# ablab/spades

Hardware: NVIDIA H100
Metric: Mk-mers/s (extract+count+index) k=55, 150 bp reads (higher is better)
Workload: dtype u64

## Files before the change

spades_b200/csrc/count.cu:

```cuda
#include <algorithm>
#include <chrono>
#include <memory>

#include "pass_plan.h"
#include "sgpu_internal.h"

namespace sg {

__device__ __forceinline__ void prefetch_l2(const void *p) { asm volatile("prefetch.global.L2 [%0];" ::"l"(p)); }

struct ReadsSrc {
    const uint64_t *words;
    const uint64_t *offs;
    const uint32_t *lens;
    int64_t n;
    uint64_t nwords;
    int K;
    static constexpr int kIds = 24;
    static constexpr int kIdLines = 48;
    static constexpr bool kSubRanges = true;
    __device__ __forceinline__ uint64_t first_word(int64_t item) const { return offs[item]; }
    __device__ __forceinline__ uint32_t len(int64_t item) const { return lens[item]; }
    __device__ __forceinline__ void prefetch_items(int64_t item, int lane) const {
        if (lane == 0) prefetch_l2(lens + item);
// ... 213 lines not shown
        uint32_t unif = 0;
        bool staged = false;
        const bool has_next = t + kRollWarps < t1;
        const int64_t nx = (t + kRollWarps) * kRollTile;
        uint64_t next_w0 = 0;
        if (has_next) {
            next_w0 = src.first_word(nx);
            src.prefetch_items(nx, lane);
        }
        const uint32_t nunits = roll_warp_setup<BOTH>(src, item0, nitems, rw, &unif, &staged);
        uint64_t *row = ids ? reinterpret_cast<uint64_t *>(ids + tile_off[t]) : nullptr;
        for (uint32_t u = lane; u < nunits; u += 32) {
            const RollUnit q = roll_unit<BOTH>(rw, nitems, u, unif, K);
            const uint64_t *seq = staged ? static_cast<const uint64_t *>(rw.words + rw.off[q.it]) : src.words + src.first_word(item0 + q.it);
            RollState<NW> st;
            roll_init<NW>(st, seq, q.j0, K, q.cnt);
            const int nrec = BOTH ? 2 * q.cnt : q.cnt;
#pragma unroll 1
            for (int g = 0; g < Src::kIds / 4; ++g) {
                uint64_t acc = 0;
#pragma unroll
                for (int e = 0; e < 4; ++e) {
                    const int s = 4 * g + e;
                    uint32_t id = 0xffffu;
                    if (s < nrec) {
                        if (s > 0 && !(BOTH && (e & 1))) roll_next<NW>(st, K);
                        const Kmer<NW> k = BOTH ? ((e & 1) ? st.r : st.f) : kmer_is_minimal<NW>(st.f, st.r) ? st.f : st.r;
                        uint32_t part;
                        if (part_of<NW>(p, k, &part)) { atomicAdd(&hist[part], 1u); id = part; }
                    }
                    acc |= (uint64_t)id << (16 * e);
                }
                if (row) row[(size_t)u * (Src::kIds / 4) + g] = acc;
            }
        }
        if (has_next && lane < 10 && next_w0 + 16 * lane < src.nwords) prefetch_l2(src.words + next_w0 + 16 * lane);
        __syncwarp();
    }
    __syncthreads();
    uint32_t *out = blk_counts + (size_t)blockIdx.x * p.PA;
    for (uint32_t i = threadIdx.x; i < p.PA; i += blockDim.x) out[i] += hist[i];
}

static const uint32_t kABatchMin = 1024;
static_assert(kABatchMin / kRollWarps >= 32 * 2, "a warp's share of the smallest batch holds one window of a warp step");
__host__ __device__ __forceinline__ size_t abatch_offset(uint32_t PA) {
    return ((((size_t)2 * PA * 4 + 15) & ~(size_t)15) + (size_t)kRollWarps * sizeof(RollWarp) + 15) & ~(size_t)15;
}
template <int NW, bool PLANNED>
constexpr size_t abatch_rec_bytes() { return NW * sizeof(uint64_t) + (PLANNED ? sizeof(uint16_t) : sizeof(uint32_t) + sizeof(uint16_t)); }

static const uint32_t kABatchNoTag = 0xffffffffu;
static const int kABatchPartBits = 13;
template <int NW, class Src, bool BOTH>
__global__ void __launch_bounds__(kRollThreads, 2) levelA_scatter_roll_k(Src src, LevelA p, uint64_t *__restrict__ base, uint64_t *__restrict__ out,
                                                                        uint32_t row_stride, uint32_t cap) {
    extern __shared__ __align__(16) unsigned char sm_raw[];
    __shared__ uint32_t s_fill;
    __shared__ uint32_t warp_tot[kRollWarps];
    const uint32_t PA = p.PA;
    uint32_t *cur = reinterpret_cast<uint32_t *>(sm_raw);
    uint32_t *cnt = cur + PA;
    RollWarp &rw = *roll_warp_slice(sm_raw, 2 * PA);
    uint64_t *stage = reinterpret_cast<uint64_t *>(sm_raw + abatch_offset(PA));
    uint32_t *tags = reinterpret_cast<uint32_t *>(stage + (size_t)cap * NW);
    uint16_t *idx = reinterpret_cast<uint16_t *>(tags + cap);
    uint64_t *mybase = base + (size_t)blockIdx.x * row_stride;
    const uint64_t region0 = mybase[0];
    for (uint32_t i = threadIdx.x; i < PA; i += blockDim.x) { cur[i] = (uint32_t)(mybase[i] - region0); cnt[i] = 0; }
    if (threadIdx.x == 0) s_fill = 0;
    __syncthreads();
    uint64_t *const out0 = out + region0 * NW;
    const int K = p.K;
    const int lane = threadIdx.x & 31, warp = threadIdx.x >> 5;
    const uint32_t lt_mask = (1u << lane) - 1u;
    const int64_t ntiles = (src.n + kRollTile - 1) / kRollTile;
    const int64_t per = (ntiles + gridDim.x - 1) / gridDim.x;
    const int64_t t0 = (int64_t)blockIdx.x * per, t1 = min(ntiles, t0 + per);

    int64_t t = t0 + warp;
    bool need_setup = true;
    int nitems = 0;
    uint32_t nunits = 0, unif = 0;
    bool staged = false;
    uint64_t next_w0 = 0;
    int u = 0, s = 0, cnt_w = 0;
    RollState<NW> st;
    for (;;) {
        while (t < t1) {
            if (need_setup) {
                const int64_t item0 = t * kRollTile;
                nitems = (int)min((int64_t)kRollTile, src.n - item0);
                const int64_t nx = (t + kRollWarps) * kRollTile;
                if (t + kRollWarps < t1) {
                    next_w0 = src.first_word(nx);
                    src.prefetch_items(nx, lane);
                }
                nunits = roll_warp_setup<BOTH>(src, item0, nitems, rw, &unif, &staged);
                u = lane - 32; s = cnt_w = 0;
                need_setup = false;
            }
            if (s >= cnt_w && u < (int)nunits) {
                u += 32;
                if (u < (int)nunits) {
                    const RollUnit q = roll_unit<BOTH>(rw, nitems, (uint32_t)u, unif, K);
                    const uint64_t *seq = staged ? static_cast<const uint64_t *>(rw.words + rw.off[q.it]) : src.words + src.first_word(t * kRollTile + q.it);
                    roll_init<NW>(st, seq, q.j0, K, q.cnt);
                    s = 0; cnt_w = BOTH ? 2 * q.cnt : q.cnt;
                }
// ... 18 lines not shown
            const uint32_t bal = __ballot_sync(0xffffffffu, mine);
            if (bal) {
                const uint32_t n = __popc(bal);
                uint32_t b0 = 0;
                if (lane == 0) b0 = atomicAdd(&s_fill, n);
                b0 = __shfl_sync(0xffffffffu, b0, 0);
                if (b0 + n > cap) {
                    if (b0 < cap && (uint32_t)lane < cap - b0) tags[b0 + lane] = kABatchNoTag;
                    break;
                }
                if (mine) {
                    const uint32_t i = b0 + __popc(bal & lt_mask);
                    const uint32_t rank = atomicAdd(&cnt[part], 1u) & 0xffffu;
                    store_rec<NW>(stage + (size_t)i * NW, k);
                    tags[i] = (rank << kABatchPartBits) | part;
                }
            }
            if (act && ++s < cnt_w && (!BOTH || !(s & 1))) roll_next<NW>(st, K);
        }
        const bool more = __syncthreads_or(t < t1);
        const uint32_t nslots = min(s_fill, cap);
        const uint32_t own = (PA + kRollThreads - 1) / kRollThreads;
        const uint32_t j0 = min(PA, threadIdx.x * own), j1 = min(PA, j0 + own);
        uint32_t sum = 0;
        for (uint32_t j = j0; j < j1; ++j) sum += cnt[j] & 0xffffu;
        uint32_t inc = sum;
#pragma unroll
        for (int o = 1; o < 32; o <<= 1) {
            const uint32_t v = __shfl_up_sync(0xffffffffu, inc, o);
            if (lane >= o) inc += v;
        }
        if (lane == 31) warp_tot[warp] = inc;
        __syncthreads();
        uint32_t wb = 0, total = 0;
#pragma unroll
        for (int w = 0; w < kRollWarps; ++w) { const uint32_t v = warp_tot[w]; if (w < warp) wb += v; total += v; }
        uint32_t o = wb + inc - sum;
        for (uint32_t j = j0; j < j1; ++j) {
            const uint32_t c = cnt[j] & 0xffffu;
            o += c;
            cnt[j] = o << 16;
            cur[j] += c;
        }
        if (threadIdx.x == 0) s_fill = 0;
        __syncthreads();
        for (uint32_t i = threadIdx.x; i < nslots; i += kRollThreads) {
            const uint32_t tg = tags[i];
            if (tg == kABatchNoTag) continue;
            idx[(cnt[tg & ((1u << kABatchPartBits) - 1)] >> 16) - 1 - (tg >> kABatchPartBits)] = (uint16_t)i;
        }
        __syncthreads();
        for (uint32_t q = threadIdx.x; q < total; q += kRollThreads) {
            const uint32_t i = idx[q], tg = tags[i];
            const uint32_t slot = cur[tg & ((1u << kABatchPartBits) - 1)] - 1 - (tg >> kABatchPartBits);
            store_rec_stream<NW>(out0 + (size_t)slot * NW, load_rec<NW>(stage + (size_t)i * NW));
        }
        __syncthreads();
        if (!more) break;
    }
    for (uint32_t i = threadIdx.x; i < PA; i += blockDim.x) mybase[i] = region0 + cur[i];
}

template <int NW, class Src, bool BOTH>
__global__ void __launch_bounds__(kRollThreads, 2) levelA_scatter_plan_k(Src src, LevelA p, uint64_t *__restrict__ base, uint64_t *__restrict__ out,
                                                                        const uint64_t *__restrict__ tile_off, const uint16_t *__restrict__ ids,
                                                                        uint32_t id_lo, uint32_t row_stride, uint32_t q_lo, uint64_t ids_len, uint32_t cap) {
    extern __shared__ __align__(16) unsigned char sm_raw[];
    __shared__ uint32_t warp_tot[kRollWarps];
    constexpr int kR = BOTH ? 2 : 1;
    constexpr int kRowV = Src::kIds / 8;
    const uint32_t PA = p.PA;
    uint32_t *cur = reinterpret_cast<uint32_t *>(sm_raw);
    uint32_t *run = cur + PA;
    RollWarp &rw = *roll_warp_slice(sm_raw, 2 * PA);
    uint64_t *stage = reinterpret_cast<uint64_t *>(sm_raw + abatch_offset(PA));
    uint16_t *ptag = reinterpret_cast<uint16_t *>(stage + (size_t)cap * NW);
    uint64_t *mybase = base + (size_t)blockIdx.x * row_stride + q_lo;
    const uint64_t region0 = mybase[0];
    for (uint32_t i = threadIdx.x; i < PA; i += blockDim.x) { cur[i] = (uint32_t)(mybase[i] - region0); run[i] = 0; }
    __syncthreads();
    uint64_t *const out0 = out + region0 * NW;
    const int K = p.K;
    const int lane = threadIdx.x & 31, warp = threadIdx.x >> 5;
    const int64_t ntiles = (src.n + kRollTile - 1) / kRollTile;
    const int64_t per = (ntiles + gridDim.x - 1) / gridDim.x;
    const int64_t t0 = (int64_t)blockIdx.x * per, t1 = min(ntiles, t0 + per);
    const uint32_t share = cap / kRollWarps;

    int64_t pt = t0 + warp;
    int pj = 0, ps = 0;
    uint32_t pn = 0;
    bool p_enter = true;
    const ulonglong2 *prow = nullptr;
    int64_t rt = pt;
    int rj = 0, rs = 0;
    bool need_setup = true;
    int nitems = 0;
    uint32_t nunits = 0, unif = 0;
    bool staged = false;
    uint64_t next_w0 = 0;
    const ulonglong2 *row = nullptr;
    for (;;) {
        uint32_t room = share;
        while (pt < t1) {
            if (p_enter) {
                const uint64_t a = tile_off[pt], b = tile_off[pt + 1];
                if (pt + kRollWarps < t1) {
                    const uint64_t nr = tile_off[pt + kRollWarps];
                    if ((Src::kIdLines >= 32 || lane < Src::kIdLines) && nr + 64 * lane < ids_len) prefetch_l2(ids + nr + 64 * lane);
                    if (lane < Src::kIdLines - 32 && nr + 64 * (32 + lane) < ids_len) prefetch_l2(ids + nr + 64 * (32 + lane));
                }
                pn = (uint32_t)((b - a) / Src::kIds);
                prow = reinterpret_cast<const ulonglong2 *>(ids + a);
                p_enter = false;
            }
            if ((uint32_t)pj * 32 >= pn) {
                pt += kRollWarps; pj = 0; ps = 0; p_enter = true;
                continue;
            }
// ... 68 lines not shown
                __syncwarp();
                rt += kRollWarps; rj = 0; rs = 0;
                need_setup = true;
                continue;
            }
            const int end = (rt == pt && rj == pj) ? ps : Src::kIds;
            const int u = rj * 32 + lane;
            if (u < (int)nunits) {
                const RollUnit q = roll_unit<BOTH>(rw, nitems, (uint32_t)u, unif, K);
                const int s_end = min(end, BOTH ? 2 * q.cnt : q.cnt);
                if (rs < s_end) {
                    uint64_t idq[Src::kIds / 4];
#pragma unroll
                    for (int v = 0; v < kRowV; ++v) {
                        const ulonglong2 x = __ldg(row + (size_t)u * kRowV + v);
                        idq[2 * v] = x.x; idq[2 * v + 1] = x.y;
                    }
                    for (int w = 0; w < rs / 4; ++w) {
#pragma unroll
                        for (int v = 0; v + 1 < Src::kIds / 4; ++v) idq[v] = idq[v + 1];
                    }
                    idq[0] >>= 16 * (rs & 3);
                    const uint64_t *seq = staged ? static_cast<const uint64_t *>(rw.words + rw.off[q.it]) : src.words + src.first_word(rt * kRollTile + q.it);
                    RollState<NW> st;
                    roll_init<NW>(st, seq, q.j0 + rs / kR, K, q.cnt - rs / kR);
                    for (int s = rs;;) {
                        const uint32_t part = (uint32_t)(idq[0] & 0xffffu) - id_lo;
                        if (part < PA) {
                            const bool fwd = BOTH ? !(s & 1) : kmer_is_minimal<NW>(st.f, st.r);
                            Kmer<NW> k;
#pragma unroll
                            for (int j = 0; j < NW; ++j) k.w[j] = fwd ? st.f.w[j] : st.r.w[j];
                            const uint32_t pos = atomicAdd(&run[part], 1u << 16) >> 16;
                            store_rec<NW>(stage + (size_t)pos * NW, k);
                            ptag[pos] = (uint16_t)part;
                        }
                        if (++s >= s_end) break;
                        if (!BOTH || !(s & 1)) roll_next<NW>(st, K);
                        if ((s & 3) == 0) {
#pragma unroll
                            for (int v = 0; v + 1 < Src::kIds / 4; ++v) idq[v] = idq[v + 1];
                        } else {
                            idq[0] >>= 16;
                        }
                    }
                }
            }
            if (end == Src::kIds) { ++rj; rs = 0; } else rs = end;
        }
        __syncthreads();
        for (uint32_t q = threadIdx.x; q < total; q += kRollThreads) {
            const uint32_t part = ptag[q];
            const uint32_t slot = cur[part] - (run[part] >> 16) + q;
            store_rec_stream<NW>(out0 + (size_t)slot * NW, load_rec<NW>(stage + (size_t)q * NW));
        }
        if (!more) break;
    }
    for (uint32_t i = threadIdx.x; i < PA; i += blockDim.x) mybase[i] = region0 + cur[i];
}

struct Seg {
    uint64_t start;
    uint64_t len;
    uint32_t bits;
    uint32_t bb;
};

__global__ void seg_init_k(const uint64_t *__restrict__ part_start, const uint64_t *__restrict__ part_total, uint32_t PA, int rA,
                           uint32_t b_lo, Seg *__restrict__ segs) {
    uint32_t part = blockIdx.x * blockDim.x + threadIdx.x;
    if (part >= PA) return;
    Seg s;
    s.start = part_start[part]; s.len = part_total[part]; s.bits = (uint32_t)rA; s.bb = ((b_lo + (part >> rA)) << 1) | 0u;
    segs[part] = s;
}

struct Pieces {
    const uint64_t *pbase;
    const uint32_t *cnt;
    uint32_t cnt_stride, PA;
    int G;
};
static const int kMaxPieces = 1024;

__global__ void stage_rows_k(const uint32_t *__restrict__ cnt, uint32_t cnt_stride, uint32_t PA, uint64_t *__restrict__ rel, uint64_t *__restrict__ row_total) {
    __shared__ uint64_t wsum[8];
    __shared__ uint64_t carry_s;
    const uint32_t *row = cnt + (size_t)blockIdx.x * cnt_stride;
    uint64_t *out = rel + (size_t)blockIdx.x * PA;
    const int lane = threadIdx.x & 31, warp = threadIdx.x >> 5;
    if (threadIdx.x == 0) carry_s = 0;
    __syncthreads();
    for (uint32_t b = 0; b < PA; b += blockDim.x) {
        const uint32_t i = b + threadIdx.x;
        const uint64_t v = i < PA ? row[i] : 0;
        uint64_t inc = v;
#pragma unroll
        for (int o = 1; o < 32; o <<= 1) {
            uint64_t t = __shfl_up_sync(0xffffffffu, inc, o);
            if (lane >= o) inc += t;
        }
        if (lane == 31) wsum[warp] = inc;
        __syncthreads();
        uint64_t wb = 0, all = 0;
        for (int w = 0; w < 8; ++w) { if (w < warp) wb += wsum[w]; all += wsum[w]; }
        const uint64_t carry = carry_s;
        if (i < PA) out[i] = carry + wb + inc - v;
        __syncthreads();
        if (threadIdx.x == 0) carry_s = carry + all;
        __syncthreads();
    }
    if (threadIdx.x == 0) row_total[blockIdx.x] = carry_s;
}
__global__ void stage_add_k(uint64_t *__restrict__ rel, const uint64_t *__restrict__ row_start, uint32_t PA, int G) {
    const uint64_t i = (uint64_t)blockIdx.x * blockDim.x + threadIdx.x;
    if (i >= (uint64_t)G * PA) return;
    rel[i] += row_start[i / PA];
}

struct RefinePlan { uint32_t cap, target, rmax; int total_bits; };
__device__ __forceinline__ int plan_r(const RefinePlan &rp, uint64_t len, uint32_t bits) {
    if (len <= rp.cap) return 0;
    int rem = rp.total_bits - (int)bits;
    if (rem <= 0) return 0;
    uint64_t want = (len + rp.target - 1) / rp.target;
    int r = 1;
    while (r < (int)rp.rmax && (1ull << r) < want) ++r;
    return r < rem ? r : rem;
}
__global__ void refine_plan_k(const Seg *__restrict__ segs, uint64_t n, RefinePlan rp, uint32_t *__restrict__ nchild, uint32_t *__restrict__ isw, int force_all) {
    uint64_t i = (uint64_t)blockIdx.x * blockDim.x + threadIdx.x;
    if (i >= n) return;
    int r = plan_r(rp, segs[i].len, segs[i].bits);
    nchild[i] = r ? (1u << r) : 1u;
    isw[i] = (r || force_all) ? 1u : 0u;
}
__global__ void refine_copy_k(const Seg *__restrict__ segs, uint64_t n, const uint32_t *__restrict__ isw, const uint64_t *__restrict__ child_base,
                              const uint64_t *__restrict__ work_pos, Seg *__restrict__ nsegs, uint64_t *__restrict__ worklist) {
    uint64_t i = (uint64_t)blockIdx.x * blockDim.x + threadIdx.x;
    if (i >= n) return;
    if (isw[i]) worklist[work_pos[i]] = i;
    else nsegs[child_base[i]] = segs[i];
}

static const int kRThreads = 1024;
static const int kRWarps = kRThreads / 32;
static const int kRMaxBins = 2048;
template <int NW> struct RBatch {
    static const int RPT = NW == 1 ? 12 : NW == 2 ? 8 : NW == 3 ? 4 : 3;
    static const int N = RPT * kRThreads;
    static constexpr size_t smem() { return (size_t)N * (NW * sizeof(uint64_t) + sizeof(uint32_t)); }
};

template <int NW, bool PIECED>
__global__ void __launch_bounds__(kRThreads) refine_k(const Seg *__restrict__ segs, const uint64_t *__restrict__ worklist, uint64_t nwork,
                                                     const uint64_t *__restrict__ child_base, RefinePlan rp, int K,
                                                     uint64_t *__restrict__ buf0, uint64_t *__restrict__ buf1, Seg *__restrict__ nsegs,
                                                     unsigned long long *__restrict__ work_counter, Pieces pc) {
    constexpr int RPT = RBatch<NW>::RPT, N = RBatch<NW>::N;
    __shared__ uint32_t hist[kRMaxBins];
    __shared__ uint32_t run_off[kRMaxBins];
    __shared__ uint32_t run_slot[kRMaxBins];
    __shared__ uint32_t warp_tot[kRWarps];
    __shared__ unsigned long long s_w;
    __shared__ uint64_t pc_start[PIECED ? kMaxPieces : 1];
    __shared__ uint32_t pc_len[PIECED ? kMaxPieces : 1];
    extern __shared__ uint64_t sm_refine_dyn[];
    uint64_t *stage = sm_refine_dyn;
    uint32_t *stage_slot = reinterpret_cast<uint32_t *>(stage + (size_t)N * NW);
    const int lane = threadIdx.x & 31, warp = threadIdx.x >> 5;
    for (;;) {
        if (threadIdx.x == 0) s_w = atomicAdd(work_counter, 1ull);
        __syncthreads();
        const uint64_t wi = s_w;
        __syncthreads();
        if (wi >= nwork) return;
        const uint64_t si = worklist[wi];
        const Seg s = segs[si];
        const int r = plan_r(rp, s.len, s.bits);
        const uint32_t nb = 1u << r;
        const uint64_t *src = ((s.bb & 1) ? buf1 : buf0) + s.start * NW;
        uint64_t *dst = ((s.bb & 1) ? buf0 : buf1) + s.start * NW;
        if (PIECED) {
            for (int g = threadIdx.x; g < pc.G; g += blockDim.x) {
                pc_start[g] = pc.pbase[(size_t)g * pc.PA + si];
                pc_len[g] = pc.cnt[(size_t)g * pc.cnt_stride + si];
            }
        }
        for (uint32_t i = threadIdx.x; i < nb; i += blockDim.x) hist[i] = 0;
        __syncthreads();
        if (PIECED) {
            for (int g = warp; g < pc.G; g += kRWarps) {
                const uint64_t *ps = buf0 + pc_start[g] * NW;
                const uint32_t n = pc_len[g];
                uint32_t i = lane;
                for (; i + 96 < n; i += 128) {
                    const Kmer<NW> k0 = load_rec<NW>(ps + (uint64_t)i * NW), k1 = load_rec<NW>(ps + (uint64_t)(i + 32) * NW);
                    const Kmer<NW> k2 = load_rec<NW>(ps + (uint64_t)(i + 64) * NW), k3 = load_rec<NW>(ps + (uint64_t)(i + 96) * NW);
                    atomicAdd(&hist[key_bits<NW>(k0, K, (int)s.bits, r)], 1u);
                    atomicAdd(&hist[key_bits<NW>(k1, K, (int)s.bits, r)], 1u);
                    atomicAdd(&hist[key_bits<NW>(k2, K, (int)s.bits, r)], 1u);
                    atomicAdd(&hist[key_bits<NW>(k3, K, (int)s.bits, r)], 1u);
                }
                for (; i < n; i += 32) {
                    const Kmer<NW> k = load_rec<NW>(ps + (uint64_t)i * NW);
                    atomicAdd(&hist[key_bits<NW>(k, K, (int)s.bits, r)], 1u);
                }
            }
        } else {
            for (uint64_t i = threadIdx.x; i < s.len; i += blockDim.x) {
                Kmer<NW> k = load_rec<NW>(src + i * NW);
                atomicAdd(&hist[key_bits<NW>(k, K, (int)s.bits, r)], 1u);
            }
        }
        __syncthreads();
        uint32_t a = 0, b = 0;
        const uint32_t i0 = 2 * threadIdx.x;
        if (i0 < nb) { a = hist[i0]; hist[i0] = 0; }
        if (i0 + 1 < nb) { b = hist[i0 + 1]; hist[i0 + 1] = 0; }
        uint32_t v = a + b, inc = v;
#pragma unroll
        for (int o = 1; o < 32; o <<= 1) {
            uint32_t t = __shfl_up_sync(0xffffffffu, inc, o);
            if (lane >= o) inc += t;
        }
        if (lane == 31) warp_tot[warp] = inc;
        __syncthreads();
        if (warp == 0) {
            uint32_t w = warp_tot[lane], winc = w;
#pragma unroll
            for (int o = 1; o < 32; o <<= 1) {
                uint32_t t = __shfl_up_sync(0xffffffffu, winc, o);
                if (lane >= o) winc += t;
            }
            warp_tot[lane] = winc - w;
        }
        __syncthreads();
        const uint32_t ex = warp_tot[warp] + inc - v;
        const uint64_t cb = child_base[si];
        if (i0 < nb) {
            Seg c; c.start = s.start + ex; c.len = a; c.bits = s.bits + (uint32_t)r; c.bb = s.bb ^ 1u;
            nsegs[cb + i0] = c;
        }
        if (i0 + 1 < nb) {
// ... 26 lines not shown
                for (int j = 0; j < RPT; ++j) {
                    const uint64_t i = cpos + threadIdx.x + (uint64_t)kRThreads * j;
                    if (i < s.len) { rec[j] = load_rec<NW>(src + i * NW); have |= 1u << j; }
                }
                cpos += N;
            }
        };
        load_batch();
        for (;;) {
            uint32_t tag[RPT];
#pragma unroll
            for (int j = 0; j < RPT; ++j) {
                if (have >> j & 1u) {
                    const uint32_t bin = key_bits<NW>(rec[j], K, (int)s.bits, r);
                    tag[j] = (atomicAdd(&hist[bin], 1u) << 11) | bin;
                }
            }
            if (!__syncthreads_or(have)) break;
            const uint32_t c0 = i0 < nb ? hist[i0] : 0u, c1 = i0 + 1 < nb ? hist[i0 + 1] : 0u;
            const uint32_t bv = c0 + c1;
            uint32_t binc = bv;
#pragma unroll
            for (int o = 1; o < 32; o <<= 1) {
                uint32_t t = __shfl_up_sync(0xffffffffu, binc, o);
                if (lane >= o) binc += t;
            }
            if (lane == 31) warp_tot[warp] = binc;
            __syncthreads();
            uint32_t w = warp_tot[lane], winc = w;
#pragma unroll
            for (int o = 1; o < 32; o <<= 1) {
                uint32_t t = __shfl_up_sync(0xffffffffu, winc, o);
                if (lane >= o) winc += t;
            }
            const uint32_t total = __shfl_sync(0xffffffffu, winc, 31);
            const uint32_t off = __shfl_sync(0xffffffffu, winc - w, warp) + binc - bv;
            if (i0 < nb) { run_off[i0] = off; run_slot[i0] = cur0; hist[i0] = 0; cur0 += c0; }
            if (i0 + 1 < nb) { run_off[i0 + 1] = off + c0; run_slot[i0 + 1] = cur1; hist[i0 + 1] = 0; cur1 += c1; }
            __syncthreads();
#pragma unroll
            for (int j = 0; j < RPT; ++j) {
                if (have >> j & 1u) {
                    const uint32_t bin = tag[j] & (kRMaxBins - 1), rank = tag[j] >> 11;
                    const uint32_t p = run_off[bin] + rank;
                    store_rec<NW>(stage + (size_t)p * NW, rec[j]);
                    stage_slot[p] = run_slot[bin] + rank;
                }
            }
            load_batch();
            __syncthreads();
            for (uint32_t p = threadIdx.x; p < total; p += kRThreads)
                store_rec_stream<NW>(dst + (uint64_t)stage_slot[p] * NW, load_rec<NW>(stage + (size_t)p * NW));
        }
    }
}

template <int NW> struct SortCfg { static const int CAP = NW <= 2 ? 2048 : 1024; };
static const int kSThreads = 512;
static const int kSWarps = kSThreads / 32;

template <int NW>
__device__ __forceinline__ void lsd_pass(const uint64_t *A, uint64_t *Bf, uint32_t n, int K, int pos, int width, uint32_t *cnt ,
                                         uint32_t *tot ) {
    static_assert(kSThreads >= 256, "one thread per digit");
    const int lane = threadIdx.x & 31, warp = threadIdx.x >> 5;
    const uint32_t chunk = ((n + kSWarps * 32 - 1) / (kSWarps * 32)) * 32;
    const uint32_t w0 = warp * chunk;
    for (int i = threadIdx.x; i < kSWarps * 256; i += kSThreads) cnt[i] = 0;
    __syncthreads();
    for (uint32_t r = 0; r < chunk; r += 32) {
        const uint32_t i = w0 + r + lane;
        uint32_t d = 256;
        if (i < n) d = key_bits<NW>(load_rec<NW>(A + (size_t)i * NW), K, pos, width);
        const uint32_t m = __match_any_sync(0xffffffffu, d);
        if (d < 256 && (int)(__ffs(m) - 1) == lane) cnt[warp * 256 + d] += __popc(m);
        __syncwarp();
    }
    __syncthreads();
    {
        const uint32_t d = threadIdx.x;
        uint32_t run = 0, inc = 0;
        if (d < 256) {
#pragma unroll
            for (int w = 0; w < kSWarps; ++w) { uint32_t t = cnt[w * 256 + d]; cnt[w * 256 + d] = run; run += t; }
            inc = run;
#pragma unroll
            for (int o = 1; o < 32; o <<= 1) {
                uint32_t t = __shfl_up_sync(0xffffffffu, inc, o);
                if (lane >= o) inc += t;
            }
            if (lane == 31) tot[warp] = inc;
        }
        __syncthreads();
        if (d < 256) {
            uint32_t wb = 0;
            for (int w = 0; w < warp; ++w) wb += tot[w];
            const uint32_t ex = wb + inc - run;
#pragma unroll
            for (int w = 0; w < kSWarps; ++w) cnt[w * 256 + d] += ex;
        }
    }
    __syncthreads();
    for (uint32_t r = 0; r < chunk; r += 32) {
        const uint32_t i = w0 + r + lane;
        uint32_t d = 256;
        Kmer<NW> k;
// ... 393 lines not shown
struct KSetBuilder {
    Ctx *ctx;
    std::unique_ptr<KSet> ks;
    DArr<unsigned long long> d_bsz;
    int64_t first = 0;
    bool double_selfrc;
    std::unique_ptr<ResultSink> sink;
    KSetBuilder(Ctx *c, int K, int nw, int B, bool counts, bool double_selfrc_, bool on_host) : ctx(c), ks(new KSet()), double_selfrc(double_selfrc_) {
        ks->ctx = c; ks->K = K; ks->nw = nw; ks->B = B; ks->has_counts = counts; ks->on_host = on_host;
        if (on_host) sink.reset(new ResultSink(c, ks.get()));
        d_bsz.alloc(c, (size_t)B);
        SG_CUDA(cudaMemsetAsync(d_bsz.p, 0, (size_t)B * 8, c->stream));
    }
    Chunk &open(int b_lo, int b_hi, uint64_t n) {
        if (sink) sink->drain();
        ks->chunks.emplace_back();
        Chunk &ch = ks->chunks.back();
        ch.n = (int64_t)n; ch.b_lo = b_lo; ch.b_hi = b_hi; ch.first = first;
        ch.keys.alloc(ctx, (size_t)n * ks->nw + 2, true);
        if (ks->has_counts) ch.counts.alloc(ctx, (size_t)n + 1, true);
        return ch;
    }
    void close() {
        first += ks->chunks.back().n;
        if (sink) sink->push();
    }
    KSet *finish() {
        if (sink) { sink->drain(); sink.reset(); }
        const int B = ks->B;
        std::vector<unsigned long long> hb(B);
        SG_CUDA(cudaMemcpyAsync(hb.data(), d_bsz.p, (size_t)B * 8, cudaMemcpyDeviceToHost, ctx->stream));
        SG_CUDA(cudaStreamSynchronize(ctx->stream));
        ks->bsz.assign(B, 0); ks->bstart.assign(B + 1, 0);
        for (int b = 0; b < B; ++b) { ks->bsz[b] = (int64_t)hb[b]; ks->bstart[b + 1] = ks->bstart[b] + ks->bsz[b]; }
        ks->n = first;
        SG_CHECK(ks->bstart[B] == ks->n, 6, "internal: bucket sizes do not add up");
        return ks.release();
    }
};

template <int NW>
static void sort_pass(Ctx *ctx, int K, DArr<uint64_t> &X, DArr<uint64_t> &Y, const uint64_t *part_start_p, const uint64_t *part_total_p, uint32_t PA,
                      int rA_, uint32_t b_lo, int b_hi, KSetBuilder &set, Timer &tm, Trace &tr, const Pieces *pieces = nullptr) {
    constexpr int CAP = SortCfg<NW>::CAP;
    const int total_bits = 2 * K;
    cudaStream_t st = ctx->stream;
    uint64_t nsegs = PA;
    DArr<Seg> segs(ctx, nsegs);
    seg_init_k<<<div_up(PA, 256), 256, 0, st>>>(part_start_p, part_total_p, PA, rA_, b_lo, segs.p);
    ctx->launches++;
    RefinePlan rp; rp.cap = CAP; rp.target = sort_target<NW>(); rp.total_bits = total_bits;
    rp.rmax = tuning().rmax;
    DArr<unsigned long long> wcounter(ctx, 4);
    tm.start();
    uint64_t rounds = 0;
    for (int round = 0; round < 300; ++round) {
        DArr<uint32_t> nchild(ctx, nsegs + 1), isw(ctx, nsegs + 1);
        DArr<uint64_t> cbase(ctx, nsegs + 1), wpos(ctx, nsegs + 1);
        SG_CUDA(cudaMemsetAsync(nchild.p + nsegs, 0, 4, st));
        SG_CUDA(cudaMemsetAsync(isw.p + nsegs, 0, 4, st));
        const bool pieced = pieces && round == 0;
        refine_plan_k<<<div_up(nsegs, 256), 256, 0, st>>>(segs.p, nsegs, rp, nchild.p, isw.p, pieced ? 1 : 0);
        ctx->launches++;
        exclusive_scan_u32_to_u64(ctx, nchild.p, cbase.p, nsegs + 1);
        exclusive_scan_u32_to_u64(ctx, isw.p, wpos.p, nsegs + 1);
        uint64_t tot[2];
        SG_CUDA(cudaMemcpyAsync(&tot[0], cbase.p + nsegs, 8, cudaMemcpyDeviceToHost, st));
        SG_CUDA(cudaMemcpyAsync(&tot[1], wpos.p + nsegs, 8, cudaMemcpyDeviceToHost, st));
        SG_CUDA(cudaStreamSynchronize(st));
        if (tot[1] == 0) break;
        DArr<Seg> nsegs_arr(ctx, tot[0]);
        DArr<uint64_t> worklist(ctx, tot[1]);
        refine_copy_k<<<div_up(nsegs, 256), 256, 0, st>>>(segs.p, nsegs, isw.p, cbase.p, wpos.p, nsegs_arr.p, worklist.p);
        ctx->launches++;
        SG_CUDA(cudaMemsetAsync(wcounter.p, 0, 8, st));
        const int grid = (int)std::min<uint64_t>(tot[1], (uint64_t)ctx->num_sms);
        const size_t sm = RBatch<NW>::smem();
        if (pieced) {
            SG_CUDA(cudaFuncSetAttribute(refine_k<NW, true>, cudaFuncAttributeMaxDynamicSharedMemorySize, (int)sm));
            refine_k<NW, true><<<grid, kRThreads, sm, st>>>(segs.p, worklist.p, tot[1], cbase.p, rp, K, X.p, Y.p, nsegs_arr.p, wcounter.p, *pieces);
        } else {
            SG_CUDA(cudaFuncSetAttribute(refine_k<NW, false>, cudaFuncAttributeMaxDynamicSharedMemorySize, (int)sm));
            refine_k<NW, false><<<grid, kRThreads, sm, st>>>(segs.p, worklist.p, tot[1], cbase.p, rp, K, X.p, Y.p, nsegs_arr.p, wcounter.p, Pieces());
        }
        ctx->launches++;
        SG_CUDA(cudaGetLastError());
        tr.mark("refine round");
        (round == 0 ? ctx->times.refine_splits_round0 : ctx->times.refine_splits_later) += tot[0] - nsegs;
        ++rounds;
        segs = std::move(nsegs_arr);
        nsegs = tot[0];
    }
    ctx->times.refine_rounds_max = std::max(ctx->times.refine_rounds_max, rounds);
    ctx->times.refine += tm.stop();
    DArr<uint32_t> ndist(ctx, nsegs + 1);
    DArr<unsigned long long> stats(ctx, 4);
    SG_CUDA(cudaMemsetAsync(ndist.p, 0, ndist.bytes(), st));
    SG_CUDA(cudaMemsetAsync(stats.p, 0, 32, st));
    SG_CUDA(cudaMemsetAsync(wcounter.p, 0, 8, st));
    tm.start();
    {
        auto launch = [&](auto kernel, size_t smem) {
            SG_CUDA(cudaFuncSetAttribute(kernel, cudaFuncAttributeMaxDynamicSharedMemorySize, (int)smem));
            int occ = 1;
            SG_CUDA(cudaOccupancyMaxActiveBlocksPerMultiprocessor(&occ, kernel, kSThreads, smem));
            if (occ < 1) occ = 1;
            int grid = (int)std::min<uint64_t>(nsegs, (uint64_t)ctx->num_sms * occ);
            if (grid < 1) grid = 1;
            kernel<<<grid, kSThreads, smem, st>>>(segs.p, nsegs, K, X.p, Y.p, ndist.p, wcounter.p, stats.p);
        };
        launch(local_sort3_k<NW, kSortBinBits, CAP>, SortSmem<NW, kSortBinBits, CAP>::bytes);
        ctx->launches++;
        SG_CUDA(cudaGetLastError());
    }
    DArr<uint64_t> dbase(ctx, nsegs + 1);
    exclusive_scan_u32_to_u64(ctx, ndist.p, dbase.p, nsegs + 1);
    uint64_t D = 0;
    unsigned long long h_stats[4];
    SG_CUDA(cudaMemcpyAsync(&D, dbase.p + nsegs, 8, cudaMemcpyDeviceToHost, st));
    SG_CUDA(cudaMemcpyAsync(h_stats, stats.p, 32, cudaMemcpyDeviceToHost, st));
    SG_CUDA(cudaStreamSynchronize(st));
    ctx->times.local_sort += tm.stop();
    tr.mark("local sort");
    SG_CHECK(h_stats[0] == 0, 6, "internal: oversize segment with unfixed key bits reached the local sort");
    ctx->times.sort_lsd_fallbacks += h_stats[1];
    ctx->times.sort_oversize_equal += h_stats[2];
    Chunk &ch = set.open((int)b_lo, b_hi, D);
    tm.start();
    if (nsegs) {
        compact_k<NW><<<div_up((int64_t)nsegs * 32, 256), 256, 0, st>>>(segs.p, nsegs, ndist.p, dbase.p, X.p, Y.p, K, set.ks->has_counts ? 1 : 0,
                                                                     set.double_selfrc ? 1 : 0, ch.keys.p, ch.counts.p, set.d_bsz.p);
        ctx->launches++;
        SG_CUDA(cudaGetLastError());
    }
    ctx->times.compact += tm.stop();
    tr.mark("compact");
    set.close();
}

template <int NW, class Src, bool BOTH>
struct LevelAJob {
    Ctx *ctx = nullptr;
    std::vector<Src> srcs;
    int K = 0, B = 0, rA = 0, G = 0;
    int s_lo = 0, s_hi = 0;
    uint32_t PA_all = 0;
    bool use_ids = false;
// ... 55 lines not shown
static void levelA_count(LevelAJob<NW, Src, BOTH> &job, Timer &tm, Trace &tr) {
    Ctx *ctx = job.ctx;
    cudaStream_t st = ctx->stream;
    const uint32_t PA_all = job.PA_all;
    const int G = job.G;
    SG_CHECK(PA_all >= 1 && PA_all <= (uint32_t)kLevelAMaxParts, 6, "internal: level-A partition table too large");
    LevelA pa_all;
    pa_all.K = job.K; pa_all.B = (uint32_t)job.B; pa_all.b_lo = (uint32_t)job.s_lo; pa_all.b_hi = (uint32_t)job.s_hi; pa_all.rA = job.rA; pa_all.PA = PA_all;
    job.blk_counts.alloc(ctx, (size_t)G * PA_all);
    job.part_total_all.alloc(ctx, (size_t)PA_all + 1);
    job.h_part.assign(PA_all, 0);
    SG_CUDA(cudaMemsetAsync(job.blk_counts.p, 0, job.blk_counts.bytes(), st));
    job.tile_off.clear(); job.ids.clear();
    job.tile_off.resize(job.srcs.size()); job.ids.resize(job.srcs.size());
    const double free0 = (double)ctx->free_bytes();
    std::vector<uint64_t> nslots(job.srcs.size(), 0);
    uint64_t all_slots = 0;
    for (size_t si = 0; si < job.srcs.size(); ++si) {
        const Src &src = job.srcs[si];
        if (src.n == 0) continue;
        const int64_t ntiles = (src.n + kRollTile - 1) / kRollTile;
        DArr<uint32_t> ttot(ctx, (size_t)ntiles + 1);
        job.tile_off[si].alloc(ctx, (size_t)ntiles + 1);
        SG_CUDA(cudaMemsetAsync(ttot.p + ntiles, 0, 4, st));
        roll_tile_ids_k<BOTH><<<div_up(ntiles, 8), 256, 0, st>>>(src, ntiles, ttot.p);
        ctx->launches++;
        exclusive_scan_u32_to_u64(ctx, ttot.p, job.tile_off[si].p, (size_t)ntiles + 1);
        SG_CUDA(cudaMemcpyAsync(&nslots[si], job.tile_off[si].p + ntiles, 8, cudaMemcpyDeviceToHost, st));
        SG_CUDA(cudaStreamSynchronize(st));
        all_slots += nslots[si];
    }
    job.use_ids = PA_all < 0xffffu && (double)all_slots * 2.0 < free0 * 0.20;
    for (size_t si = 0; si < job.srcs.size(); ++si) {
        if (!job.use_ids) job.tile_off[si] = DArr<uint64_t>();
        else if (job.srcs[si].n) job.ids[si].alloc(ctx, (size_t)nslots[si] + 8);
    }
    tm.start();
    SG_CUDA(cudaFuncSetAttribute(levelA_count_roll_k<NW, Src, BOTH>, cudaFuncAttributeMaxDynamicSharedMemorySize, (int)roll_smem_bytes(PA_all)));
    job.for_each_src([&](size_t si, const Src &src) {
        levelA_count_roll_k<NW, Src, BOTH><<<G, kRollThreads, roll_smem_bytes(PA_all), st>>>(src, pa_all, job.blk_counts.p, job.tile_off[si].p, job.ids[si].p);
        ctx->launches++;
    });
    SG_CUDA(cudaGetLastError());
    levelA_totals_k<<<div_up(PA_all, 256), 256, 0, st>>>(job.blk_counts.p, PA_all, G, job.part_total_all.p);
    ctx->launches++;
    SG_CUDA(cudaMemcpyAsync(job.h_part.data(), job.part_total_all.p, (size_t)PA_all * 8, cudaMemcpyDeviceToHost, st));
    SG_CUDA(cudaStreamSynchronize(st));
    ctx->times.extract_count += tm.stop();
    tr.mark("A1 count+totals");
}

template <int NW, class Src, bool BOTH>
static void levelA_scatter(LevelAJob<NW, Src, BOTH> &job, int b_lo, int b_hi, uint64_t I_pass, uint64_t total_records, uint64_t *X, uint64_t *pbase_buf,
                           Pieces &pcs, Timer &tm, Trace &tr) {
    Ctx *ctx = job.ctx;
    cudaStream_t st = ctx->stream;
    const int G = job.G;
    const uint32_t PA_all = job.PA_all;
    const uint32_t p_lo = (uint32_t)(b_lo - job.s_lo) << job.rA;
    LevelA pa;
    pa.K = job.K; pa.B = (uint32_t)job.B; pa.b_lo = (uint32_t)b_lo; pa.b_hi = (uint32_t)b_hi; pa.rA = job.rA; pa.PA = (uint32_t)(b_hi - b_lo) << job.rA;
    const uint32_t PA = pa.PA;
    SG_CHECK(PA >= 1 && PA <= (uint32_t)kLevelAMaxParts && G <= kMaxPieces, 6, "internal: level-A pass geometry");
    DArr<uint64_t> base(ctx, (size_t)G * PA);
    {
        DArr<uint64_t> row_total(ctx, (size_t)G + 1), row_start(ctx, (size_t)G + 1);
        SG_CUDA(cudaMemsetAsync(row_total.p + G, 0, 8, st));
        stage_rows_k<<<G, 256, 0, st>>>(job.blk_counts.p + p_lo, PA_all, PA, base.p, row_total.p);
        exclusive_scan_u64(ctx, row_total.p, row_start.p, (size_t)G + 1);
        stage_add_k<<<div_up((int64_t)G * PA, 256), 256, 0, st>>>(base.p, row_start.p, PA, G);
        ctx->launches += 2;
        SG_CUDA(cudaMemcpyAsync(pbase_buf, base.p, (size_t)G * PA * 8, cudaMemcpyDeviceToDevice, st));
    }
    pcs.pbase = pbase_buf; pcs.cnt = job.blk_counts.p + p_lo; pcs.cnt_stride = PA_all; pcs.PA = PA; pcs.G = G;
    tm.start();
    int nsub_auto = (int)(4.0 * (double)I_pass / (double)std::max<uint64_t>(1, total_records) + 0.5);
    nsub_auto = std::min(4, std::max(1, nsub_auto));
    uint32_t nsub = job.use_ids && !BOTH && Src::kSubRanges ? (uint32_t)(tuning().a_sub ? tuning().a_sub : nsub_auto) : 1u;
    if (nsub > PA) nsub = PA;
    for (uint32_t sb = 0; sb < nsub; ++sb) {
        const uint32_t q_lo = (uint32_t)((uint64_t)PA * sb / nsub), q_hi = (uint32_t)((uint64_t)PA * (sb + 1) / nsub);
        if (q_hi == q_lo) continue;
        LevelA pa_sub = pa;
        pa_sub.PA = q_hi - q_lo;
        uint32_t cap = 0;
        const size_t smem = job.use_ids ? levelA_batch_smem<NW, true>(pa_sub.PA, &cap) : levelA_batch_smem<NW, false>(pa_sub.PA, &cap);
        if (job.use_ids) SG_CUDA(cudaFuncSetAttribute(levelA_scatter_plan_k<NW, Src, BOTH>, cudaFuncAttributeMaxDynamicSharedMemorySize, (int)smem));
        else SG_CUDA(cudaFuncSetAttribute(levelA_scatter_roll_k<NW, Src, BOTH>, cudaFuncAttributeMaxDynamicSharedMemorySize, (int)smem));
        job.for_each_src([&](size_t si, const Src &src) {
            if (job.use_ids)
                levelA_scatter_plan_k<NW, Src, BOTH><<<G, kRollThreads, smem, st>>>(src, pa_sub, base.p, X, job.tile_off[si].p, job.ids[si].p, p_lo + q_lo, PA, q_lo, (uint64_t)job.ids[si].n, cap);
            else
                levelA_scatter_roll_k<NW, Src, BOTH><<<G, kRollThreads, smem, st>>>(src, pa, base.p, X, PA, cap);
            ctx->launches++; ctx->times.level_a_scatters++;
        });
    }
    SG_CUDA(cudaGetLastError());
    ctx->times.extract_scatter += tm.stop();
    tr.mark("A2 scatter");
}

static double pass_bytes_needed(uint64_t recs, size_t W) { return (double)recs * W * 2.0 + (double)recs * (W + 4) * 0.6 + (64 << 20); }

template <int NW, bool BOTH, class Src>
static void run_count(Ctx *ctx, const std::vector<Src> &srcs, int K, uint64_t est_records, KSetBuilder &set, ChunkStager *stage = nullptr) {
    const int total_bits = 2 * K, B = set.ks->B;
    const size_t W = 8 * NW;
    cudaStream_t st = ctx->stream;
    Timer tm(st);
    Trace tr("sgpu count", st);

    const int rA = levelA_key_bits(est_records, B, total_bits, sort_target<NW>(), tuning().pa_max);
    ctx->times.level_a_key_bits = (uint64_t)rA;
    const int SR = std::max(1, kLevelAMaxParts >> rA);
    const int n_ranges = (B + SR - 1) / SR;
    for (int s_lo = 0; s_lo < B; s_lo += SR) {
        const int share = (kMaxChunks - (int)set.ks->chunks.size()) / (n_ranges - s_lo / SR);
        LevelAJob<NW, Src, BOTH> job;
        job.ctx = ctx; job.srcs = srcs; job.K = K; job.B = B; job.rA = rA; job.G = ctx->num_sms * levelA_ctas_per_sm(); job.stage = stage;
        job.s_lo = s_lo; job.s_hi = std::min(B, s_lo + SR);
        job.PA_all = (uint32_t)(job.s_hi - job.s_lo) << rA;
        levelA_count(job, tm, tr);
        std::vector<uint64_t> before(job.s_hi - job.s_lo + 1, 0);
        for (int b = job.s_lo; b < job.s_hi; ++b) before[b - job.s_lo + 1] = before[b - job.s_lo] + job.bucket_records(b);
        PassPlan plan(job.s_lo, job.s_hi, share, std::move(before));
        const uint64_t total_records = plan.records(job.s_lo, job.s_hi);
        auto need = [&](int a, int b) { return pass_bytes_needed(plan.records(a, b), W); };
        plan.aim((double)ctx->budget_left(), set.sink != nullptr, need, [&](int a, int b) { return (double)plan.records(a, b) * (W + 4) * 0.5; });
        while (!plan.done()) {
            const int b_lo = plan.bounds.back(), b_hi = plan.next((double)ctx->budget_left(), need);
            const uint64_t I = plan.records(b_lo, b_hi);
            const uint32_t p_lo = (uint32_t)(b_lo - job.s_lo) << rA;
            const uint32_t PA = (uint32_t)(b_hi - b_lo) << rA;
            DArr<uint64_t> part_total(ctx, PA + 1), part_start(ctx, PA + 1);
            SG_CUDA(cudaMemcpyAsync(part_total.p, job.part_total_all.p + p_lo, (size_t)PA * 8, cudaMemcpyDeviceToDevice, st));
            SG_CUDA(cudaMemsetAsync(part_total.p + PA, 0, 8, st));
            exclusive_scan_u64(ctx, part_total.p, part_start.p, PA + 1);
            ctx->times.passes++;
            ctx->times.instances += I;
            DArr<uint64_t> X(ctx, (size_t)I * NW + 2), Y(ctx, (size_t)I * NW + 2);
            DArr<uint64_t> pbase(ctx, (size_t)job.G * PA);
            Pieces pcs;
            levelA_scatter(job, b_lo, b_hi, I, total_records, X.p, pbase.p, pcs, tm, tr);
            sort_pass<NW>(ctx, K, X, Y, part_start.p, part_total.p, PA, rA, (uint32_t)b_lo, b_hi, set, tm, tr, &pcs);
        }
    }
}

__global__ void count_windows_k(const uint32_t *__restrict__ lens, int64_t n, int K, unsigned long long *__restrict__ out) {
    unsigned long long s = 0;
    for (int64_t i = (int64_t)blockIdx.x * blockDim.x + threadIdx.x; i < n; i += (int64_t)gridDim.x * blockDim.x) {
        int L = (int)lens[i];
        if (L >= K) s += (unsigned long long)(L - K + 1);
    }
    for (int o = 16; o; o >>= 1) s += __shfl_down_sync(0xffffffffu, s, o);
    if ((threadIdx.x & 31) == 0 && s) atomicAdd(out, s);
}

static uint64_t count_windows(Ctx *ctx, int K) {
    DArr<unsigned long long> d_w(ctx, 1);
    SG_CUDA(cudaMemsetAsync(d_w.p, 0, 8, ctx->stream));
    if (ctx->n_reads) {
        count_windows_k<<<ctx->num_sms * 4, 256, 0, ctx->stream>>>(ctx->d_lens, ctx->n_reads, K, d_w.p);
        ctx->launches++;
    }
    unsigned long long wn = 0;
    SG_CUDA(cudaMemcpyAsync(&wn, d_w.p, 8, cudaMemcpyDeviceToHost, ctx->stream));
    SG_CUDA(cudaStreamSynchronize(ctx->stream));
    return (uint64_t)wn;
}

static ReadsSrc reads_source(Ctx *ctx, int K) {
    ReadsSrc src;
    src.words = ctx->d_words; src.offs = ctx->d_offs; src.lens = ctx->d_lens; src.n = ctx->n_reads; src.nwords = ctx->n_words; src.K = K;
    return src;
}

template <int NW>
static KSet *count_reads_nw(Ctx *ctx, int K, int B, int mode, bool on_host) {
    ensure_reads_on_device(ctx);
    const uint64_t wn = count_windows(ctx, K);
    std::vector<ReadsSrc> srcs{reads_source(ctx, K)};
    const bool canonical = mode == kCanonical;
    KSetBuilder set(ctx, K, NW, B, canonical, canonical && K % 2 == 0, on_host);
    if (canonical) run_count<NW, false>(ctx, srcs, K, wn, set);
    else run_count<NW, true>(ctx, srcs, K, wn * 2, set);
    return set.finish();
}

KSet *count_from_reads(Ctx *ctx, int K, int B, int mode, bool result_on_host) {
    SG_CHECK(K >= 1 && K <= 128, 2, "K must be in [1,128]");
    SG_CHECK(B >= 1 && B <= (1 << 20), 2, "num_buckets must be in [1, 2^20]");
    ctx->times = PhaseTimes();
    switch (nwords_of(K)) {
        case 1: return count_reads_nw<1>(ctx, K, B, mode, result_on_host);
        case 2: return count_reads_nw<2>(ctx, K, B, mode, result_on_host);
// ... 484 lines not shown
```

Measured before the change: 8709.

## Build next-digit histograms during level-A scatter to skip refine's piece histogram pass

The level-A scatter kernels now atomically count, per partition, the next dw key bits of each record into a global digits table. The first refinement round then builds its bin histogram from this table instead of re-reading every scattered record piece. This is meant to remove a full read pass over the pass buffer at the cost of global atomics during scatter and an extra PA<<dw table. It also adds a device-side consistency flag with a host sync and a partition-size check.

```diff
diff --git a/spades_b200/csrc/count.cu b/spades_b200/csrc/count.cu
--- a/spades_b200/csrc/count.cu
+++ b/spades_b200/csrc/count.cu
@@ -289,9 +289,13 @@
 
 static const uint32_t kABatchNoTag = 0xffffffffu;
 static const int kABatchPartBits = 13;
+template <int NW>
+__device__ __forceinline__ uint32_t next_digit(const Kmer<NW> &k, int K, int rA, int w) {
+    return w ? (uint32_t)(k.w[0] >> ((NW == 1 ? 2 * K : 64) - rA - w)) & ((1u << w) - 1u) : 0u;
+}
 template <int NW, class Src, bool BOTH>
 __global__ void __launch_bounds__(kRollThreads, 2) levelA_scatter_roll_k(Src src, LevelA p, uint64_t *__restrict__ base, uint64_t *__restrict__ out,
-                                                                        uint32_t row_stride, uint32_t cap) {
+                                                                        uint32_t row_stride, uint32_t cap, uint32_t *__restrict__ digits, int dw) {
     extern __shared__ __align__(16) unsigned char sm_raw[];
     __shared__ uint32_t s_fill;
     __shared__ uint32_t warp_tot[kRollWarps];
@@ -416,8 +420,11 @@
         __syncthreads();
         for (uint32_t q = threadIdx.x; q < total; q += kRollThreads) {
             const uint32_t i = idx[q], tg = tags[i];
-            const uint32_t slot = cur[tg & ((1u << kABatchPartBits) - 1)] - 1 - (tg >> kABatchPartBits);
-            store_rec_stream<NW>(out0 + (size_t)slot * NW, load_rec<NW>(stage + (size_t)i * NW));
+            const uint32_t part = tg & ((1u << kABatchPartBits) - 1);
+            const uint32_t slot = cur[part] - 1 - (tg >> kABatchPartBits);
+            const Kmer<NW> k = load_rec<NW>(stage + (size_t)i * NW);
+            store_rec_stream<NW>(out0 + (size_t)slot * NW, k);
+            if (digits) atomicAdd(&digits[((size_t)part << dw) | next_digit<NW>(k, K, p.rA, dw)], 1u);
         }
         __syncthreads();
         if (!more) break;
@@ -428,7 +435,8 @@
 template <int NW, class Src, bool BOTH>
 __global__ void __launch_bounds__(kRollThreads, 2) levelA_scatter_plan_k(Src src, LevelA p, uint64_t *__restrict__ base, uint64_t *__restrict__ out,
                                                                         const uint64_t *__restrict__ tile_off, const uint16_t *__restrict__ ids,
-                                                                        uint32_t id_lo, uint32_t row_stride, uint32_t q_lo, uint64_t ids_len, uint32_t cap) {
+                                                                        uint32_t id_lo, uint32_t row_stride, uint32_t q_lo, uint64_t ids_len, uint32_t cap,
+                                                                        uint32_t *__restrict__ digits, int dw) {
     extern __shared__ __align__(16) unsigned char sm_raw[];
     __shared__ uint32_t warp_tot[kRollWarps];
     constexpr int kR = BOTH ? 2 : 1;
@@ -603,7 +611,9 @@
         for (uint32_t q = threadIdx.x; q < total; q += kRollThreads) {
             const uint32_t part = ptag[q];
             const uint32_t slot = cur[part] - (run[part] >> 16) + q;
-            store_rec_stream<NW>(out0 + (size_t)slot * NW, load_rec<NW>(stage + (size_t)q * NW));
+            const Kmer<NW> k = load_rec<NW>(stage + (size_t)q * NW);
+            store_rec_stream<NW>(out0 + (size_t)slot * NW, k);
+            if (digits) atomicAdd(&digits[((size_t)(q_lo + part) << dw) | next_digit<NW>(k, K, p.rA, dw)], 1u);
         }
         if (!more) break;
     }
@@ -629,8 +639,9 @@
 struct Pieces {
     const uint64_t *pbase;
     const uint32_t *cnt;
+    const uint32_t *digits;
     uint32_t cnt_stride, PA;
-    int G;
+    int G, dw;
 };
 static const int kMaxPieces = 1024;
 
@@ -707,7 +718,7 @@
 __global__ void __launch_bounds__(kRThreads) refine_k(const Seg *__restrict__ segs, const uint64_t *__restrict__ worklist, uint64_t nwork,
                                                      const uint64_t *__restrict__ child_base, RefinePlan rp, int K,
                                                      uint64_t *__restrict__ buf0, uint64_t *__restrict__ buf1, Seg *__restrict__ nsegs,
-                                                     unsigned long long *__restrict__ work_counter, Pieces pc) {
+                                                     unsigned long long *__restrict__ work_counter, Pieces pc, uint32_t *__restrict__ bad) {
     constexpr int RPT = RBatch<NW>::RPT, N = RBatch<NW>::N;
     __shared__ uint32_t hist[kRMaxBins];
     __shared__ uint32_t run_off[kRMaxBins];
@@ -740,7 +751,13 @@
         }
         for (uint32_t i = threadIdx.x; i < nb; i += blockDim.x) hist[i] = 0;
         __syncthreads();
-        if (PIECED) {
+        if (PIECED && pc.digits) {
+            const uint32_t *dg = pc.digits + (si << pc.dw);
+            for (uint32_t e = threadIdx.x; e < (1u << pc.dw); e += blockDim.x) {
+                const uint32_t v = dg[e];
+                if (v) atomicAdd(&hist[e >> (pc.dw - r)], v);
+            }
+        } else if (PIECED) {
             for (int g = warp; g < pc.G; g += kRWarps) {
                 const uint64_t *ps = buf0 + pc_start[g] * NW;
                 const uint32_t n = pc_len[g];
@@ -873,6 +890,7 @@
             for (uint32_t p = threadIdx.x; p < total; p += kRThreads)
                 store_rec_stream<NW>(dst + (uint64_t)stage_slot[p] * NW, load_rec<NW>(stage + (size_t)p * NW));
         }
+        if ((i0 < nb && cur0 != ex + a) || (i0 + 1 < nb && cur1 != ex + a + b)) *bad = 1u;
     }
 }
 
@@ -1372,6 +1390,8 @@
     RefinePlan rp; rp.cap = CAP; rp.target = sort_target<NW>(); rp.total_bits = total_bits;
     rp.rmax = tuning().rmax;
     DArr<unsigned long long> wcounter(ctx, 4);
+    DArr<uint32_t> bad(ctx, 1);
+    SG_CUDA(cudaMemsetAsync(bad.p, 0, 4, st));
     tm.start();
     uint64_t rounds = 0;
     for (int round = 0; round < 300; ++round) {
@@ -1398,10 +1418,10 @@
         const size_t sm = RBatch<NW>::smem();
         if (pieced) {
             SG_CUDA(cudaFuncSetAttribute(refine_k<NW, true>, cudaFuncAttributeMaxDynamicSharedMemorySize, (int)sm));
-            refine_k<NW, true><<<grid, kRThreads, sm, st>>>(segs.p, worklist.p, tot[1], cbase.p, rp, K, X.p, Y.p, nsegs_arr.p, wcounter.p, *pieces);
+            refine_k<NW, true><<<grid, kRThreads, sm, st>>>(segs.p, worklist.p, tot[1], cbase.p, rp, K, X.p, Y.p, nsegs_arr.p, wcounter.p, *pieces, bad.p);
         } else {
             SG_CUDA(cudaFuncSetAttribute(refine_k<NW, false>, cudaFuncAttributeMaxDynamicSharedMemorySize, (int)sm));
-            refine_k<NW, false><<<grid, kRThreads, sm, st>>>(segs.p, worklist.p, tot[1], cbase.p, rp, K, X.p, Y.p, nsegs_arr.p, wcounter.p, Pieces());
+            refine_k<NW, false><<<grid, kRThreads, sm, st>>>(segs.p, worklist.p, tot[1], cbase.p, rp, K, X.p, Y.p, nsegs_arr.p, wcounter.p, Pieces(), bad.p);
         }
         ctx->launches++;
         SG_CUDA(cudaGetLastError());
@@ -1413,6 +1433,10 @@
     }
     ctx->times.refine_rounds_max = std::max(ctx->times.refine_rounds_max, rounds);
     ctx->times.refine += tm.stop();
+    uint32_t h_bad = 0;
+    SG_CUDA(cudaMemcpyAsync(&h_bad, bad.p, 4, cudaMemcpyDeviceToHost, st));
+    SG_CUDA(cudaStreamSynchronize(st));
+    SG_CHECK(h_bad == 0, 6, "internal: refinement child sizes do not match the records");
     DArr<uint32_t> ndist(ctx, nsegs + 1);
     DArr<unsigned long long> stats(ctx, 4);
     SG_CUDA(cudaMemsetAsync(ndist.p, 0, ndist.bytes(), st));
@@ -1574,7 +1598,7 @@
 
 template <int NW, class Src, bool BOTH>
 static void levelA_scatter(LevelAJob<NW, Src, BOTH> &job, int b_lo, int b_hi, uint64_t I_pass, uint64_t total_records, uint64_t *X, uint64_t *pbase_buf,
-                           Pieces &pcs, Timer &tm, Trace &tr) {
+                           Pieces &pcs, Timer &tm, Trace &tr, uint32_t *digits = nullptr, int dw = 0) {
     Ctx *ctx = job.ctx;
     cudaStream_t st = ctx->stream;
     const int G = job.G;
@@ -1595,6 +1619,7 @@
         SG_CUDA(cudaMemcpyAsync(pbase_buf, base.p, (size_t)G * PA * 8, cudaMemcpyDeviceToDevice, st));
     }
     pcs.pbase = pbase_buf; pcs.cnt = job.blk_counts.p + p_lo; pcs.cnt_stride = PA_all; pcs.PA = PA; pcs.G = G;
+    pcs.digits = digits; pcs.dw = dw;
     tm.start();
     int nsub_auto = (int)(4.0 * (double)I_pass / (double)std::max<uint64_t>(1, total_records) + 0.5);
     nsub_auto = std::min(4, std::max(1, nsub_auto));
@@ -1611,9 +1636,10 @@
         else SG_CUDA(cudaFuncSetAttribute(levelA_scatter_roll_k<NW, Src, BOTH>, cudaFuncAttributeMaxDynamicSharedMemorySize, (int)smem));
         job.for_each_src([&](size_t si, const Src &src) {
             if (job.use_ids)
-                levelA_scatter_plan_k<NW, Src, BOTH><<<G, kRollThreads, smem, st>>>(src, pa_sub, base.p, X, job.tile_off[si].p, job.ids[si].p, p_lo + q_lo, PA, q_lo, (uint64_t)job.ids[si].n, cap);
+                levelA_scatter_plan_k<NW, Src, BOTH><<<G, kRollThreads, smem, st>>>(src, pa_sub, base.p, X, job.tile_off[si].p, job.ids[si].p, p_lo + q_lo, PA, q_lo, (uint64_t)job.ids[si].n, cap,
+                                                                                           digits, dw);
             else
-                levelA_scatter_roll_k<NW, Src, BOTH><<<G, kRollThreads, smem, st>>>(src, pa, base.p, X, PA, cap);
+                levelA_scatter_roll_k<NW, Src, BOTH><<<G, kRollThreads, smem, st>>>(src, pa, base.p, X, PA, cap, digits, dw);
             ctx->launches++; ctx->times.level_a_scatters++;
         });
     }
@@ -1643,6 +1669,7 @@
         job.s_lo = s_lo; job.s_hi = std::min(B, s_lo + SR);
         job.PA_all = (uint32_t)(job.s_hi - job.s_lo) << rA;
         levelA_count(job, tm, tr);
+        SG_CHECK(*std::max_element(job.h_part.begin(), job.h_part.end()) <= 0xffffffffull, 6, "internal: a level-A partition holds 2^32 records or more");
         std::vector<uint64_t> before(job.s_hi - job.s_lo + 1, 0);
         for (int b = job.s_lo; b < job.s_hi; ++b) before[b - job.s_lo + 1] = before[b - job.s_lo] + job.bucket_records(b);
         PassPlan plan(job.s_lo, job.s_hi, share, std::move(before));
@@ -1662,8 +1689,14 @@
             ctx->times.instances += I;
             DArr<uint64_t> X(ctx, (size_t)I * NW + 2), Y(ctx, (size_t)I * NW + 2);
             DArr<uint64_t> pbase(ctx, (size_t)job.G * PA);
+            const int dw = std::min<int>((int)tuning().rmax, total_bits - rA);
+            DArr<uint32_t> digits;
+            if (!BOTH && NW >= 2) {
+                digits.alloc(ctx, (size_t)PA << dw);
+                SG_CUDA(cudaMemsetAsync(digits.p, 0, digits.bytes(), st));
+            }
             Pieces pcs;
-            levelA_scatter(job, b_lo, b_hi, I, total_records, X.p, pbase.p, pcs, tm, tr);
+            levelA_scatter(job, b_lo, b_hi, I, total_records, X.p, pbase.p, pcs, tm, tr, digits.p, dw);
             sort_pass<NW>(ctx, K, X, Y, part_start.p, part_total.p, PA, rA, (uint32_t)b_lo, b_hi, set, tm, tr, &pcs);
         }
     }
```

After: 8958, median of 6. +2.9%, better.
